# thedonutfactory/rs-tfhe

Hardware: AMD Instinct MI355X
Metric: gate-bootstraps/sec (hom_nand, SECURITY_128_BIT) (higher is better)
Workload: dtype f64

## Files before the change

rs-tfhe_amd/csrc/blind_rotate.hpp:

```cpp
#pragma once
#include "fft512.hpp"

namespace tfhe {


template <typename P>
__device__ __forceinline__ uint32_t rot_read(const P *p, int j, int k) {
  int idx = (j - k) & (2 * kN - 1);
  uint32_t v = p[idx & (kN - 1)];
  return (idx & kN) ? ~v : v;
}

using f64x2 = __attribute__((ext_vector_type(2))) double;
using u32x4 = __attribute__((ext_vector_type(4))) unsigned int;

__device__ __forceinline__ f64x2 ldkey(__amdgpu_buffer_rsrc_t rsrc, uint32_t lane_off, uint32_t soff) {
  if (TFHE_ABL_NOKEY) {
    f64x2 r;
    r.x = (double)(lane_off + soff);
    r.y = (double)(lane_off ^ soff);
    return r;
  }
  u32x4 v = __builtin_amdgcn_raw_buffer_load_b128(rsrc, (int)lane_off, (int)soff, 0);
  return __builtin_bit_cast(f64x2, v);
}

#ifndef TFHE_PREFETCH_A
#define TFHE_PREFETCH_A 8
#endif
#ifndef TFHE_PREFETCH_B
#define TFHE_PREFETCH_B 4
#endif
#ifndef TFHE_L1_PA
#define TFHE_L1_PA 7
#endif
#ifndef TFHE_RELOAD_I3
#define TFHE_RELOAD_I3 1
#endif
#ifndef TFHE_INV_PAIR
#define TFHE_INV_PAIR 1
#endif

__device__ __forceinline__ int32_t sbfe(uint32_t src, int shift, int width) {
  int32_t d;
  asm("v_bfe_i32 %0, %1, %2, %3" : "=v"(d) : "v"(src), "s"(shift), "v"(width));
  return d;
}

#ifndef TFHE_WG_WAVES
#define TFHE_WG_WAVES 4
#endif
#ifndef TFHE_WG_SYNC
#define TFHE_WG_SYNC 1
#endif
template <int LEVEL>
__device__ __forceinline__ void wg_sync() {
  if (TFHE_WG_WAVES > 1 && TFHE_WG_SYNC >= LEVEL) __builtin_amdgcn_s_barrier();
}

#ifndef TFHE_ACC_LDS_ADD
#define TFHE_ACC_LDS_ADD 1
#endif
__device__ __forceinline__ void acc_add(uint32_t *p, uint32_t v) {
#if TFHE_ACC_LDS_ADD
  __hip_atomic_fetch_add(p, v, __ATOMIC_RELAXED, __HIP_MEMORY_SCOPE_WORKGROUP);
#else
  *p += v;
#endif
}

template <bool INIT>
__device__ __forceinline__ void cmac(double &fr, double &fi, double xr, double xi, f64x2 v) {
  if (INIT) {
    fr = xr * v.x;
    fi = xr * v.y;
  } else {
    fr = fma(xr, v.x, fr);
    fi = fma(xr, v.y, fi);
  }
  fr = fma(-xi, v.y, fr);
  fi = fma(xi, v.x, fi);
}

template <int L, bool INIT>
__device__ __forceinline__ void external_product_row(int r, int shift, const uint32_t (&w_lo)[8],
                                                     const uint32_t (&w_hi)[8], __amdgpu_buffer_rsrc_t bsk_rsrc,
                                                     uint32_t bsk_i_off, const Twiddles &tw, double2 *tile,
                                                     int lane, int bgbit, double (&fa_re)[8], double (&fa_im)[8],
                                                     double (&fb_re)[8], double (&fb_im)[8]) {
  const uint32_t lane_off = (uint32_t)lane * 16u;
  wg_sync<3>();
  const uint32_t row_off = bsk_i_off + (uint32_t)r * (2u * kN2 * 16u);
  f64x2 va[8], vb[8];
  constexpr int PA = (L == 1 && TFHE_PREFETCH_A > TFHE_L1_PA) ? TFHE_L1_PA : TFHE_PREFETCH_A;
  constexpr int PB = TFHE_PREFETCH_B;
#pragma unroll
  for (int s = 0; s < PA; ++s) va[s] = ldkey(bsk_rsrc, lane_off, row_off + (uint32_t)s * 1024u);
#pragma unroll
  for (int s = 0; s < PB; ++s) vb[s] = ldkey(bsk_rsrc, lane_off, row_off + (uint32_t)(kN2 * 16 + s * 1024));
  double re[8], im[8];
#pragma unroll
  for (int m = 0; m < 8; ++m) {
    re[m] = (double)sbfe(w_lo[m], shift, bgbit);
    im[m] = (double)sbfe(w_hi[m], shift, bgbit);
  }
  fft_forward(re, im, tw, tile, lane);
#pragma unroll
  for (int s = PA; s < 8; ++s) va[s] = ldkey(bsk_rsrc, lane_off, row_off + (uint32_t)s * 1024u);
#pragma unroll
  for (int s = PB; s < 8; ++s) vb[s] = ldkey(bsk_rsrc, lane_off, row_off + (uint32_t)(kN2 * 16 + s * 1024));
#pragma unroll
  for (int s = 0; s < 8; ++s) cmac<INIT>(fa_re[s], fa_im[s], re[s], im[s], va[s]);
#pragma unroll
  for (int s = 0; s < 8; ++s) cmac<INIT>(fb_re[s], fb_im[s], re[s], im[s], vb[s]);
}

template <int L, bool INIT0>
__device__ __forceinline__ void external_product_half(int half_sel, const uint32_t (&t_lo)[8],
                                                      const uint32_t (&t_hi)[8],
                                                      __amdgpu_buffer_rsrc_t bsk_rsrc, uint32_t bsk_i_off,
                                                      const Twiddles &tw, double2 *tile, int lane, int bgbit,
                                                      uint32_t signmask, double (&fa_re)[8],
                                                      double (&fa_im)[8], double (&fb_re)[8],
                                                      double (&fb_im)[8]) {
  uint32_t w_lo[8], w_hi[8];
#pragma unroll
  for (int m = 0; m < 8; ++m) {
    w_lo[m] = t_lo[m] ^ signmask;
    w_hi[m] = t_hi[m] ^ signmask;
  }
  if (TFHE_WG_SYNC == 2) wg_sync<2>();
  external_product_row<L, INIT0>(half_sel * L, 32 - bgbit, w_lo, w_hi, bsk_rsrc, bsk_i_off, tw, tile, lane, bgbit,
                                 fa_re, fa_im, fb_re, fb_im);
  int rows = L;
  if (L > 1) asm volatile("" : "+s"(rows));
#pragma unroll 1
  for (int i = 1; i < rows; ++i)
    external_product_row<L, false>(half_sel * L + i, 32 - (i + 1) * bgbit, w_lo, w_hi, bsk_rsrc, bsk_i_off, tw, tile,
                                   lane, bgbit, fa_re, fa_im, fb_re, fb_im);
}

struct BlindRotateArgs {
  const uint32_t *in_a;
  const uint32_t *in_b;
  uint32_t ca, cb, cconst;
  const uint8_t *gate_codes;
  const uint32_t *idx_a;
  const uint32_t *idx_b;
  const uint32_t *testvec;
  size_t per_ct_stride;
  const double2 *bsk;
  const double2 *tw;
  int n, bgbit;
  uint32_t offset;
  uint32_t *out_trlwe;
  uint32_t *out_lv1;
  uint32_t *out_ext2;
  size_t count;
  unsigned long long *clk;
  uint32_t *err_flag;
  int lut_shift, n_luts;
  size_t out_fn_stride;
};

__device__ constexpr uint32_t kGateCa[11] = {0xFFFFFFFFu, 1u, 1u, 1u, 1u, 0xFFFFFFFFu, 0xFFFFFFFFu, 1u, 0xFFFFFFFFu, 1u, 1u};
__device__ constexpr uint32_t kGateCb[11] = {0xFFFFFFFFu, 1u, 1u, 2u, 0xFFFFFFFEu, 0xFFFFFFFFu, 1u, 0xFFFFFFFFu, 1u, 0xFFFFFFFFu, 0u};
__device__ constexpr uint32_t kGateCc[11] = {0x20000000u, 0x20000000u, 0xE0000000u, 0x40000000u, 0xC0000000u, 0xE0000000u,
                                             0xE0000000u, 0xE0000000u, 0x20000000u, 0x20000000u, 0u};

constexpr int kAccBytes = 2 * kN * 4;
constexpr int kBrWaves = TFHE_WG_WAVES;
__host__ __device__ __forceinline__ size_t blind_rotate_wave_lds_bytes(int n) {
  return ((size_t)kTileBytes + kAccBytes + (size_t)n * 2 + 15) & ~(size_t)15;
}
__host__ __device__ __forceinline__ size_t blind_rotate_lds_bytes(int n) {
  return kBrWaves * blind_rotate_wave_lds_bytes(n) + kT2Bytes;
}
constexpr int kStageLdsBytes = kTileBytes + kT2Bytes;

template <int L, bool FAST, bool MANY>
__device__ __forceinline__ void blind_rotate_batch(BlindRotateArgs A) {
  extern __shared__ __attribute__((aligned(16))) unsigned char smem_wg[];
  const int n = A.n;
  const int lane = threadIdx.x & 63;
  const int wave = kBrWaves > 1 ? __builtin_amdgcn_readfirstlane(threadIdx.x >> 6) : 0;
  unsigned char *smem = smem_wg + (size_t)wave * blind_rotate_wave_lds_bytes(n);
  double2 *tile = reinterpret_cast<double2 *>(smem);
  uint32_t *acc = reinterpret_cast<uint32_t *>(smem + kTileBytes);
  uint16_t *s_abar = reinterpret_cast<uint16_t *>(smem + kTileBytes + kAccBytes);
  double2 *t2tab = reinterpret_cast<double2 *>(smem_wg + (size_t)kBrWaves * blind_rotate_wave_lds_bytes(n));
  size_t ct = (size_t)blockIdx.x * kBrWaves + wave;
  const bool live = ct < A.count;
  if (!live) ct = A.count - 1;
  const unsigned long long clk0 = A.clk ? __builtin_amdgcn_s_memtime() : 0ull;
  const unsigned long long rtc0 = A.clk ? __builtin_amdgcn_s_memrealtime() : 0ull;

  Twiddles tw;
  tw.load<TFHE_ABL_TW_REL && !MANY>(A.tw, t2tab, lane);

  uint32_t gca = A.ca, gcb = A.cb, gcc = A.cconst;
  if (A.gate_codes) {
    uint32_t code = A.gate_codes[ct];
    if (code > 10u) {
      if (A.err_flag && lane == 0) atomicOr(A.err_flag, 1u);
      code = 10u;
    }
    gca = kGateCa[code];
    gcb = kGateCb[code];
    gcc = kGateCc[code];
  }
  const uint32_t *pa = A.in_a + (A.idx_a ? (size_t)A.idx_a[ct] : ct) * (size_t)(n + 1);
  const uint32_t *pb = (A.in_b && gcb) ? A.in_b + (A.idx_b ? (size_t)A.idx_b[ct] : ct) * (size_t)(n + 1) : nullptr;
  const int dl = MANY ? A.lut_shift : 0;
  for (int i = lane; i < n; i += 64) {
    uint32_t p = gca * pa[i];
    if (pb) p += gcb * pb[i];
    s_abar[i] = (uint16_t)(((uint32_t)(p + (1u << (20 + dl))) >> (21 + dl)) << dl);
  }
  uint32_t pbody = gca * pa[n];
  if (pb) pbody += gcb * pb[n];
  pbody += gcc;
  const int b_tilda = 2 * kN - (int)((((uint64_t)pbody + (1ull << (20 + dl))) >> (21 + dl)) << dl);

  const uint32_t *tv = A.testvec + ct * A.per_ct_stride;
#pragma unroll
  for (int m = 0; m < 16; ++m) {
    int j = lane + 64 * m;
    acc[j] = rot_read(tv, j, b_tilda);
    acc[kN + j] = rot_read(tv + kN, j, b_tilda);
  }
  __syncthreads();

  constexpr uint32_t per_i_bytes = 2u * L * 2u * kN2 * 16u;
  const __amdgpu_buffer_rsrc_t bsk_rsrc =
      __builtin_amdgcn_make_buffer_rsrc((void *)A.bsk, 0, (int)((uint32_t)n * per_i_bytes), 0x00020000);
  const uint32_t offset = A.offset;
  uint32_t signmask = 0;
#pragma unroll
  for (int i = 0; i < L; ++i) signmask |= 1u << (32 - i * A.bgbit - 1);
#pragma unroll 1
  for (int i = 0; i < n; ++i) {
    wg_sync<1>();
    const int k = s_abar[i];
    double fa_re[8], fa_im[8], fb_re[8], fb_im[8];
    {
      uint32_t t_lo[8], t_hi[8];
#pragma unroll
      for (int m = 0; m < 8; ++m) {
        const int j = lane + 64 * m;
        t_lo[m] = rot_read(acc, j, k) - acc[j] + offset;
        t_hi[m] = rot_read(acc, j + kN2, k) - acc[j + kN2] + offset;
      }
      external_product_half<L, true>(0, t_lo, t_hi, bsk_rsrc, (uint32_t)i * per_i_bytes, tw, tile, lane, A.bgbit,
                                     signmask, fa_re, fa_im, fb_re, fb_im);
    }
    {
      const uint32_t *p = acc + kN;
      uint32_t t_lo[8], t_hi[8];
#pragma unroll
      for (int m = 0; m < 8; ++m) {
        const int j = lane + 64 * m;
        t_lo[m] = rot_read(p, j, k) - p[j] + offset;
        t_hi[m] = rot_read(p, j + kN2, k) - p[j + kN2] + offset;
      }
      external_product_half<L, false>(1, t_lo, t_hi, bsk_rsrc, (uint32_t)i * per_i_bytes, tw, tile, lane, A.bgbit,
                                      signmask, fa_re, fa_im, fb_re, fb_im);
    }
#if TFHE_RELOAD_I3
    {
      int z = 0;
      asm volatile("" : "+v"(z));
      tw.reload_i3(A.tw, lane, z);
    }
#endif
#if TFHE_INV_PAIR
    fft_inverse2(fa_re, fa_im, fb_re, fb_im, tw, tile, lane);
#pragma unroll
    for (int m = 0; m < 8; ++m) {
      const int j = lane + 64 * m;
      acc_add(&acc[j], round_product<FAST>(fa_re[m]));
      acc_add(&acc[j + kN2], round_product<FAST>(fa_im[m]));
      acc_add(&acc[kN + j], round_product<FAST>(fb_re[m]));
      acc_add(&acc[kN + j + kN2], round_product<FAST>(fb_im[m]));
    }
#else
    fft_inverse(fa_re, fa_im, tw, tile, lane);
#pragma unroll
    for (int m = 0; m < 8; ++m) {
      const int j = lane + 64 * m;
      acc[j] += round_product<FAST>(fa_re[m]);
      acc[j + kN2] += round_product<FAST>(fa_im[m]);
    }
    fft_inverse(fb_re, fb_im, tw, tile, lane);
#pragma unroll
    for (int m = 0; m < 8; ++m) {
      const int j = lane + 64 * m;
      acc[kN + j] += round_product<FAST>(fb_re[m]);
      acc[kN + j + kN2] += round_product<FAST>(fb_im[m]);
    }
#endif
    wave_lds_sync();
  }

  if (!live) return;
  if (A.out_trlwe) {
    uint32_t *o = A.out_trlwe + ct * (size_t)(2 * kN);
#pragma unroll
    for (int m = 0; m < 32; ++m) o[lane + 64 * m] = acc[lane + 64 * m];
  }
  if constexpr (MANY) {
    for (int j = 0; j < A.n_luts; ++j) {
      const size_t row = (size_t)j * A.out_fn_stride + ct;
      if (A.out_lv1) {
        uint32_t *o = A.out_lv1 + row * (size_t)(kN + 1);
#pragma unroll
        for (int m = 0; m < 16; ++m) {
          const int i = lane + 64 * m;
          o[i] = i <= j ? acc[j - i] : ~acc[kN + j - i];
        }
        if (lane == 0) o[kN] = acc[kN + j];
      }
      if (A.out_ext2) {
        uint32_t *o = A.out_ext2 + row * (size_t)(n + 1);
        for (int i = lane; i < n; i += 64) o[i] = i <= j ? acc[j - i] : ~acc[n + j - i];
        if (lane == 0) o[n] = acc[kN + j];
      }
    }
  } else {
    if (A.out_lv1) {
      uint32_t *o = A.out_lv1 + ct * (size_t)(kN + 1);
#pragma unroll
      for (int m = 0; m < 16; ++m) {
        const int i = lane + 64 * m;
        o[i] = i == 0 ? acc[0] : ~acc[kN - i];
      }
      if (lane == 0) o[kN] = acc[kN];
    }
    if (A.out_ext2) {
      uint32_t *o = A.out_ext2 + ct * (size_t)(n + 1);
      for (int i = lane; i < n; i += 64) o[i] = i == 0 ? acc[0] : ~acc[n - i];
      if (lane == 0) o[n] = acc[kN];
    }
  }
  if (A.clk && lane == 0) {
    atomicAdd(&A.clk[0], __builtin_amdgcn_s_memtime() - clk0);
    atomicAdd(&A.clk[1], __builtin_amdgcn_s_memrealtime() - rtc0);
  }
}

template <int L, bool FAST>
__global__ __launch_bounds__(64 * kBrWaves, 2) void k_blind_rotate(BlindRotateArgs A) {
  blind_rotate_batch<L, FAST, false>(A);
}
template <int L, bool FAST>
__global__ __launch_bounds__(64 * kBrWaves, 2) void k_blind_rotate_many(BlindRotateArgs A) {
  blind_rotate_batch<L, FAST, true>(A);
}

__global__ void k_tlwe_lincomb(uint32_t ca, const uint32_t *__restrict__ a, uint32_t cb,
                               const uint32_t *__restrict__ b, uint32_t cconst, uint32_t *__restrict__ out,
                               uint32_t width, size_t total) {
  const size_t idx = (size_t)blockIdx.x * blockDim.x + threadIdx.x;
  if (idx >= total) return;
  uint32_t v = ca * a[idx];
  if (b) v += cb * b[idx];
  if (idx % width == width - 1) v += cconst;
  out[idx] = v;
}


template <int L, bool FAST>
__global__ __launch_bounds__(64) void k_external_product(const uint32_t *in, const int32_t *bsk_index,
                                                          const double2 *bsk, uint32_t bsk_bytes,
                                                          const double2 *twt, int bgbit, uint32_t offset,
                                                          uint32_t *out) {
  extern __shared__ __attribute__((aligned(16))) unsigned char smem[];
  double2 *tile = reinterpret_cast<double2 *>(smem);
  const int lane = threadIdx.x;
  const size_t ct = blockIdx.x;
  Twiddles tw;
  tw.load(twt, reinterpret_cast<double2 *>(smem + kTileBytes), lane);
  constexpr uint32_t per_i_bytes = 2u * L * 2u * kN2 * 16u;
  const __amdgpu_buffer_rsrc_t bsk_rsrc =
      __builtin_amdgcn_make_buffer_rsrc((void *)bsk, 0, (int)bsk_bytes, 0x00020000);
  const uint32_t idx = (uint32_t)__builtin_amdgcn_readfirstlane(bsk_index[ct]);
  uint32_t signmask = 0;
#pragma unroll
  for (int i = 0; i < L; ++i) signmask |= 1u << (32 - i * bgbit - 1);
  double fa_re[8], fa_im[8], fb_re[8], fb_im[8];
  {
    const uint32_t *p = in + ct * (size_t)(2 * kN);
    uint32_t t_lo[8], t_hi[8];
#pragma unroll
    for (int m = 0; m < 8; ++m) {
      t_lo[m] = p[lane + 64 * m] + offset;
      t_hi[m] = p[lane + 64 * m + kN2] + offset;
    }
    external_product_half<L, true>(0, t_lo, t_hi, bsk_rsrc, idx * per_i_bytes, tw, tile, lane, bgbit, signmask,
                                   fa_re, fa_im, fb_re, fb_im);
  }
  {
    const uint32_t *p = in + ct * (size_t)(2 * kN) + kN;
    uint32_t t_lo[8], t_hi[8];
#pragma unroll
    for (int m = 0; m < 8; ++m) {
      t_lo[m] = p[lane + 64 * m] + offset;
      t_hi[m] = p[lane + 64 * m + kN2] + offset;
    }
    external_product_half<L, false>(1, t_lo, t_hi, bsk_rsrc, idx * per_i_bytes, tw, tile, lane, bgbit, signmask,
                                    fa_re, fa_im, fb_re, fb_im);
  }
  uint32_t *o = out + ct * (size_t)(2 * kN);
  fft_inverse(fa_re, fa_im, tw, tile, lane);
#pragma unroll
  for (int m = 0; m < 8; ++m) {
    o[lane + 64 * m] = round_product<FAST>(fa_re[m]);
    o[lane + 64 * m + kN2] = round_product<FAST>(fa_im[m]);
  }
  fft_inverse(fb_re, fb_im, tw, tile, lane);
#pragma unroll
  for (int m = 0; m < 8; ++m) {
    o[kN + lane + 64 * m] = round_product<FAST>(fb_re[m]);
    o[kN + lane + 64 * m + kN2] = round_product<FAST>(fb_im[m]);
  }
}

__global__ __launch_bounds__(64) void k_ifft(const uint32_t *src, const double2 *twt, double *res) {
  extern __shared__ __attribute__((aligned(16))) unsigned char smem[];
  double2 *tile = reinterpret_cast<double2 *>(smem);
  const int lane = threadIdx.x;
  const size_t p = blockIdx.x;
  Twiddles tw;
  tw.load(twt, reinterpret_cast<double2 *>(smem + kTileBytes), lane);
  double re[8], im[8];
#pragma unroll
  for (int m = 0; m < 8; ++m) {
    re[m] = (double)(int32_t)src[p * kN + lane + 64 * m];
    im[m] = (double)(int32_t)src[p * kN + lane + 64 * m + kN2];
  }
  fft_forward(re, im, tw, tile, lane);
#pragma unroll
  for (int s = 0; s < 8; ++s) {
    int k = bin_of(lane, s);
    res[p * kN + k] = re[s] * 2.0;
    res[p * kN + k + kN2] = im[s] * 2.0;
  }
}

__global__ __launch_bounds__(64) void k_fft(const double *src, const double2 *twt, uint32_t *res) {
  extern __shared__ __attribute__((aligned(16))) unsigned char smem[];
  double2 *tile = reinterpret_cast<double2 *>(smem);
  const int lane = threadIdx.x;
  const size_t p = blockIdx.x;
  Twiddles tw;
  tw.load(twt, reinterpret_cast<double2 *>(smem + kTileBytes), lane);
  double re[8], im[8];
#pragma unroll
  for (int s = 0; s < 8; ++s) {
    int k = bin_of(lane, s);
    re[s] = src[p * kN + k] * 0x1p-10;
    im[s] = src[p * kN + k + kN2] * 0x1p-10;
  }
  fft_inverse(re, im, tw, tile, lane);
#pragma unroll
  for (int m = 0; m < 8; ++m) {
    res[p * kN + lane + 64 * m] = round_half_away_to_torus(re[m]);
    res[p * kN + lane + 64 * m + kN2] = round_half_away_to_torus(im[m]);
  }
}

__global__ __launch_bounds__(64) void k_poly_mul(const uint32_t *a, const uint32_t *b,
                                                  const double2 *twt, uint32_t *res) {
  extern __shared__ __attribute__((aligned(16))) unsigned char smem[];
  double2 *tile = reinterpret_cast<double2 *>(smem);
  const int lane = threadIdx.x;
  const size_t p = blockIdx.x;
  Twiddles tw;
  tw.load(twt, reinterpret_cast<double2 *>(smem + kTileBytes), lane);
  double are[8], aim[8], bre[8], bim[8];
#pragma unroll
  for (int m = 0; m < 8; ++m) {
    are[m] = (double)(int32_t)a[p * kN + lane + 64 * m];
    aim[m] = (double)(int32_t)a[p * kN + lane + 64 * m + kN2];
    bre[m] = (double)(int32_t)b[p * kN + lane + 64 * m];
    bim[m] = (double)(int32_t)b[p * kN + lane + 64 * m + kN2];
  }
  fft_forward(are, aim, tw, tile, lane);
  fft_forward(bre, bim, tw, tile, lane);
#pragma unroll
  for (int s = 0; s < 8; ++s) {
    double r = (are[s] * bre[s] - aim[s] * bim[s]) * 0x1p-9;
    double i = (are[s] * bim[s] + aim[s] * bre[s]) * 0x1p-9;
    are[s] = r;
    aim[s] = i;
  }
  fft_inverse(are, aim, tw, tile, lane);
#pragma unroll
  for (int m = 0; m < 8; ++m) {
    res[p * kN + lane + 64 * m] = round_half_away_to_torus(are[m]);
    res[p * kN + lane + 64 * m + kN2] = round_half_away_to_torus(aim[m]);
  }
}

__global__ void k_sample_extract(const uint32_t *trlwe, int k, uint32_t *out, size_t count) {
  size_t ct = blockIdx.x;
  const uint32_t *a = trlwe + ct * (size_t)(2 * kN);
  uint32_t *o = out + ct * (size_t)(kN + 1);
  for (int i = threadIdx.x; i <= kN; i += blockDim.x) {
    if (i == kN)
      o[kN] = a[kN + k];
    else if (i <= k)
      o[i] = a[k - i];
    else
      o[i] = ~a[kN + k - i];
  }
}

__global__ void k_bsk_convert(const double *ref, double2 *eng, size_t polys, double scale ) {
  size_t p = blockIdx.x;
  int t = threadIdx.x;
  int s = t >> 6, mu = t & 63;
  int k = bin_of(mu, s);
  eng[p * kN2 + t] = make_double2(ref[p * kN + k] * scale, ref[p * kN + k + kN2] * scale);
}

}
```

rs-tfhe_amd/csrc/experiment.hpp:

```cpp
#pragma once
#if (defined(TFHE_ABL_NOKEY) && TFHE_ABL_NOKEY) || (defined(TFHE_ABL_NOLDS) && TFHE_ABL_NOLDS) || \
    (defined(TFHE_ABL_NOFFT) && TFHE_ABL_NOFFT) || (defined(TFHE_ABL_TPB_DPP) && TFHE_ABL_TPB_DPP) || \
    (defined(TFHE_ABL_KM_NOBARRIER) && TFHE_ABL_KM_NOBARRIER) || (defined(TFHE_ABL_LAT) && TFHE_ABL_LAT) || \
    (defined(TFHE_ABL_SL) && TFHE_ABL_SL) || (defined(TFHE_ABL_ROUND_LSB) && TFHE_ABL_ROUND_LSB) || \
    (defined(TFHE_ABL_TW_REL) && TFHE_ABL_TW_REL)
#ifndef TFHE_EXPERIMENT
#error "TFHE_ABL_* are timing-only experiment switches (results wrong by construction): build with -DTFHE_EXPERIMENT (profiles/exp/build_variants.sh)"
#endif
#define TFHE_ABLATED 1
#else
#define TFHE_ABLATED 0
#endif
#ifndef TFHE_ABL_NOKEY
#define TFHE_ABL_NOKEY 0
#endif
#ifndef TFHE_ABL_NOLDS
#define TFHE_ABL_NOLDS 0
#endif
#ifndef TFHE_ABL_NOFFT
#define TFHE_ABL_NOFFT 0
#endif
#ifndef TFHE_ABL_TPB_DPP
#define TFHE_ABL_TPB_DPP 0
#endif
#ifndef TFHE_ABL_LAT
#define TFHE_ABL_LAT 0
#endif
#ifndef TFHE_ABL_ROUND_LSB
#define TFHE_ABL_ROUND_LSB 0
#endif
#ifndef TFHE_ABL_TW_REL
#define TFHE_ABL_TW_REL 0
#endif
#ifndef TFHE_ABL_KM_NOBARRIER
#define TFHE_ABL_KM_NOBARRIER 0
#endif
#ifndef TFHE_ABL_SL
#define TFHE_ABL_SL 0
#endif
```

rs-tfhe_amd/csrc/fft512.hpp:

```cpp
#pragma once
#ifndef TFHE_FFT_HOST_EMU
#include <hip/hip_runtime.h>
#endif
#include <stdint.h>

#include "experiment.hpp"

namespace tfhe {

constexpr int kN = 1024;
constexpr int kN2 = 512;
constexpr int kPlane = 72;
constexpr int kTileCplx = 8 * kPlane;
constexpr int kTileBytes = kTileCplx * 16;

__device__ constexpr double kCmRe[8] = {1.0,
                                        0.98078528040323044912618223613424,
                                        0.92387953251128675612818318939679,
                                        0.83146961230254523707878837761791,
                                        0.70710678118654752440084436210485,
                                        0.55557023301960222474283081394853,
                                        0.38268343236508977172845998403040,
                                        0.19509032201612826784828486847702};
__device__ constexpr double kCmIm[8] = {0.0,
                                        0.19509032201612826784828486847702,
                                        0.38268343236508977172845998403040,
                                        0.55557023301960222474283081394853,
                                        0.70710678118654752440084436210485,
                                        0.83146961230254523707878837761791,
                                        0.92387953251128675612818318939679,
                                        0.98078528040323044912618223613424};

constexpr int kTwEntries = 640;
constexpr int kT2Bytes = 64 * 16;
struct Twiddles {
  double f3[8];
  double i3[10];
  const double2 *t2;
  template <bool SKEW = false>
  __device__ __forceinline__ void load(const double2 *__restrict__ tw, double2 *t2_lds, int lane) {
#pragma unroll
    for (int q = 0; q < 4; ++q) {
      double2 a = tw[q * 64 + lane];
      f3[2 * q] = a.x;
      f3[2 * q + 1] = a.y;
    }
#pragma unroll
    for (int q = 0; q < 5; ++q) {
      double2 a = tw[256 + q * 64 + lane];
      i3[2 * q] = a.x;
      i3[2 * q + 1] = a.y;
    }
#if TFHE_ABL_TW_REL
    if (SKEW) {
      double2 e = tw[576 + lane];
      const double k = lane == 49 ? 1.0 + 0x1p-47 : 1.0;
      e.x *= k;
      e.y *= k;
      t2_lds[lane] = e;
    } else
#endif
    t2_lds[lane] = tw[576 + lane];
    t2 = t2_lds;
    __syncthreads();
  }
  __device__ __forceinline__ void reload_i3(const double2 *__restrict__ tw, int lane, int opaque_zero) {
#pragma unroll
    for (int q = 0; q < 5; ++q) {
      double2 a = tw[256 + q * 64 + lane + opaque_zero];
      i3[2 * q] = a.x;
      i3[2 * q + 1] = a.y;
    }
  }
};

template <bool INV>
__device__ __forceinline__ void dft8(double (&re)[8], double (&im)[8]) {
  if (TFHE_ABL_NOFFT) return;
  constexpr double H = 0.70710678118654752440084436210485;
  double a0r = re[0] + re[4], a0i = im[0] + im[4];
  double a4r = re[0] - re[4], a4i = im[0] - im[4];
  double a1r = re[1] + re[5], a1i = im[1] + im[5];
  double t5r = re[1] - re[5], t5i = im[1] - im[5];
  double a2r = re[2] + re[6], a2i = im[2] + im[6];
  double t6r = re[2] - re[6], t6i = im[2] - im[6];
  double a3r = re[3] + re[7], a3i = im[3] + im[7];
  double t7r = re[3] - re[7], t7i = im[3] - im[7];
  double p5r, p5i, a6r, a6i, p7r, p7i;
  if (!INV) {
    p5r = t5r + t5i;  p5i = t5i - t5r;
    a6r = t6i;        a6i = -t6r;
    p7r = t7i - t7r;  p7i = -(t7r + t7i);
  } else {
    p5r = t5r - t5i;  p5i = t5r + t5i;
    a6r = -t6i;       a6i = t6r;
    p7r = -(t7r + t7i);  p7i = t7r - t7i;
  }
  double b0r = a0r + a2r, b0i = a0i + a2i;
  double b2r = a0r - a2r, b2i = a0i - a2i;
  double b1r = a1r + a3r, b1i = a1i + a3i;
  double u3r = a1r - a3r, u3i = a1i - a3i;
  double b3r, b3i;
  if (!INV) { b3r = u3i; b3i = -u3r; } else { b3r = -u3i; b3i = u3r; }
  double b4r = a4r + a6r, b4i = a4i + a6i;
  double b6r = a4r - a6r, b6i = a4i - a6i;
  double q5r = p5r + p7r, q5i = p5i + p7i;
  double u7r = p5r - p7r, u7i = p5i - p7i;
  double q7r, q7i;
  if (!INV) { q7r = u7i; q7i = -u7r; } else { q7r = -u7i; q7i = u7r; }
  re[0] = b0r + b1r; im[0] = b0i + b1i;
  re[4] = b0r - b1r; im[4] = b0i - b1i;
  re[2] = b2r + b3r; im[2] = b2i + b3i;
  re[6] = b2r - b3r; im[6] = b2i - b3i;
  re[1] = fma(H, q5r, b4r);  im[1] = fma(H, q5i, b4i);
  re[5] = fma(-H, q5r, b4r); im[5] = fma(-H, q5i, b4i);
  re[3] = fma(H, q7r, b6r);  im[3] = fma(H, q7i, b6i);
  re[7] = fma(-H, q7r, b6r); im[7] = fma(-H, q7i, b6i);
}

template <bool CONJ>
__device__ __forceinline__ void cmul(double &xr, double &xi, double wr, double wi) {
  double r, i;
  if (!CONJ) {
    r = xr * wr - xi * wi;
    i = xr * wi + xi * wr;
  } else {
    r = xr * wr + xi * wi;
    i = xi * wr - xr * wi;
  }
  xr = r;
  xi = i;
}

__device__ __forceinline__ void bfly(double &ar, double &ai, double &br, double &bi, double wr, double wi) {
  const double xr = fma(-wi, bi, fma(wr, br, ar));
  const double xi = fma(wi, br, fma(wr, bi, ai));
  br = fma(2.0, ar, -xr);
  bi = fma(2.0, ai, -xi);
  ar = xr;
  ai = xi;
}

template <bool INV, bool SCALE = false>
__device__ __forceinline__ void sdft8(double (&re)[8], double (&im)[8], double c4r, double c4i, double c2r,
                                      double c2i, double c1r, double c1i, double cwr, double cwi,
                                      double gr = 1.0, double gi = 0.0) {
  if (TFHE_ABL_NOFFT) return;
  if (SCALE) {
    cmul<false>(re[0], im[0], gr, gi);
    cmul<false>(re[2], im[2], gr, gi);
    cmul<false>(re[1], im[1], gr, gi);
    cmul<false>(re[3], im[3], gr, gi);
  }
  bfly(re[0], im[0], re[4], im[4], c4r, c4i);
  bfly(re[2], im[2], re[6], im[6], c4r, c4i);
  bfly(re[1], im[1], re[5], im[5], c4r, c4i);
  bfly(re[3], im[3], re[7], im[7], c4r, c4i);
  bfly(re[0], im[0], re[2], im[2], c2r, c2i);
  bfly(re[1], im[1], re[3], im[3], c2r, c2i);
  if (!INV) {
    bfly(re[4], im[4], re[6], im[6], c2i, -c2r);
    bfly(re[5], im[5], re[7], im[7], c2i, -c2r);
  } else {
    bfly(re[4], im[4], re[6], im[6], -c2i, c2r);
    bfly(re[5], im[5], re[7], im[7], -c2i, c2r);
  }
  bfly(re[0], im[0], re[1], im[1], c1r, c1i);
  bfly(re[4], im[4], re[5], im[5], cwr, cwi);
  if (!INV) {
    bfly(re[2], im[2], re[3], im[3], c1i, -c1r);
    bfly(re[6], im[6], re[7], im[7], cwi, -cwr);
  } else {
    bfly(re[2], im[2], re[3], im[3], -c1i, c1r);
    bfly(re[6], im[6], re[7], im[7], -cwi, cwr);
  }
  const double r1 = re[4], i1 = im[4], r3 = re[6], i3 = im[6], r4 = re[1], i4 = im[1], r6 = re[3], i6 = im[3];
  re[1] = r1; im[1] = i1;
  re[3] = r3; im[3] = i3;
  re[4] = r4; im[4] = i4;
  re[6] = r6; im[6] = i6;
}

__device__ __forceinline__ void wave_lds_sync() { asm volatile("s_waitcnt lgkmcnt(0)" ::: "memory"); }
__device__ __forceinline__ void wave_lds_order() { asm volatile("" ::: "memory"); }
constexpr double kP1c4 = 0.70710678118654752440084436210485;

#if !defined(TFHE_FFT_HOST_EMU) && TFHE_ABL_TPB_DPP
__device__ __forceinline__ void abl_crosslane_exchange(double (&re)[8], double (&im)[8]) {
  uint32_t w[32];
#pragma unroll
  for (int i = 0; i < 8; ++i) {
    w[4 * i] = (uint32_t)__double2loint(re[i]);
    w[4 * i + 1] = (uint32_t)__double2hiint(re[i]);
    w[4 * i + 2] = (uint32_t)__double2loint(im[i]);
    w[4 * i + 3] = (uint32_t)__double2hiint(im[i]);
  }
#pragma unroll
  for (int i = 0; i < 16; ++i) asm volatile("v_permlane32_swap_b32 %0, %1" : "+v"(w[i]), "+v"(w[i + 16]));
#pragma unroll
  for (int i = 0; i < 16; ++i) asm volatile("v_permlane16_swap_b32 %0, %1" : "+v"(w[2 * i]), "+v"(w[2 * i + 1]));
#pragma unroll
  for (int i = 0; i < 16; ++i) {
    uint32_t t;
    asm volatile("v_mov_b32_dpp %0, %1 row_ror:8 row_mask:0xf bank_mask:0x3" : "=v"(t) : "v"(w[i]), "0"(w[i + 16]));
    asm volatile("v_mov_b32_dpp %0, %1 row_ror:8 row_mask:0xf bank_mask:0xc" : "+v"(w[i]) : "v"(w[i + 16]));
    asm volatile("v_mov_b32_dpp %0, %1 quad_perm:[0,1,2,3] row_mask:0xf bank_mask:0x3" : "+v"(w[i + 16]) : "v"(t));
  }
#pragma unroll
  for (int i = 0; i < 8; ++i) {
    re[i] = __hiloint2double((int)w[4 * i + 1], (int)w[4 * i]);
    im[i] = __hiloint2double((int)w[4 * i + 3], (int)w[4 * i + 2]);
  }
}
#endif

__device__ __forceinline__ void tpA_write(const double (&re)[8], const double (&im)[8], double2 *tile, int lane) {
  if (TFHE_ABL_NOLDS) return;
#pragma unroll
  for (int k = 0; k < 8; ++k) tile[k * kPlane + lane] = make_double2(re[k], im[k]);
}
__device__ __forceinline__ void tpA_read(double (&re)[8], double (&im)[8], const double2 *tile, int lane) {
  if (TFHE_ABL_NOLDS) return;
  const int hi = lane >> 3, lo = lane & 7;
#pragma unroll
  for (int s = 0; s < 8; ++s) {
    double2 v = tile[hi * kPlane + lo + 8 * s];
    re[s] = v.x;
    im[s] = v.y;
  }
}
__device__ __forceinline__ void tpB_write(const double (&re)[8], const double (&im)[8], double2 *tile, int lane) {
  if (TFHE_ABL_NOLDS || TFHE_ABL_TPB_DPP) return;
  const int hi = lane >> 3, lo = lane & 7;
#pragma unroll
  for (int k = 0; k < 8; ++k) tile[hi * kPlane + k * 9 + lo] = make_double2(re[k], im[k]);
}
__device__ __forceinline__ void tpB_read(double (&re)[8], double (&im)[8], const double2 *tile, int lane) {
  if (TFHE_ABL_NOLDS) return;
#if !defined(TFHE_FFT_HOST_EMU) && TFHE_ABL_TPB_DPP
  abl_crosslane_exchange(re, im);
  return;
#endif
  const int hi = lane >> 3, lo = lane & 7;
#pragma unroll
  for (int s = 0; s < 8; ++s) {
    double2 v = tile[hi * kPlane + lo * 9 + s];
    re[s] = v.x;
    im[s] = v.y;
  }
}
__device__ __forceinline__ void tpBi_write(const double (&re)[8], const double (&im)[8], double2 *tile, int lane) {
  if (TFHE_ABL_NOLDS || TFHE_ABL_TPB_DPP) return;
  const int hi = lane >> 3, lo = lane & 7;
#pragma unroll
  for (int s = 0; s < 8; ++s) tile[hi * kPlane + lo * 9 + s] = make_double2(re[s], im[s]);
}
__device__ __forceinline__ void tpBi_read(double (&re)[8], double (&im)[8], const double2 *tile, int lane) {
  if (TFHE_ABL_NOLDS) return;
#if !defined(TFHE_FFT_HOST_EMU) && TFHE_ABL_TPB_DPP
  abl_crosslane_exchange(re, im);
  return;
#endif
  const int hi = lane >> 3, lo = lane & 7;
#pragma unroll
  for (int k = 0; k < 8; ++k) {
    double2 v = tile[hi * kPlane + k * 9 + lo];
    re[k] = v.x;
    im[k] = v.y;
  }
}
__device__ __forceinline__ void tpAi_write(const double (&re)[8], const double (&im)[8], double2 *tile, int lane) {
  if (TFHE_ABL_NOLDS) return;
  const int hi = lane >> 3, lo = lane & 7;
#pragma unroll
  for (int s = 0; s < 8; ++s) tile[hi * kPlane + lo + 8 * s] = make_double2(re[s], im[s]);
}
__device__ __forceinline__ void tpAi_read(double (&re)[8], double (&im)[8], const double2 *tile, int lane) {
  if (TFHE_ABL_NOLDS) return;
#pragma unroll
  for (int k = 0; k < 8; ++k) {
    double2 v = tile[k * kPlane + lane];
    re[k] = v.x;
    im[k] = v.y;
  }
}

__device__ __forceinline__ void fwd_pass1(double (&re)[8], double (&im)[8]) {
  sdft8<false>(re, im, kP1c4, kP1c4, kCmRe[2], kCmIm[2], kCmRe[1], kCmIm[1], kCmRe[3], -kCmIm[3]);
}
__device__ __forceinline__ void fwd_pass2(double (&re)[8], double (&im)[8], const Twiddles &tw, int lane) {
  const int hi = lane >> 3;
  const double2 c4 = tw.t2[hi], c2 = tw.t2[8 + hi], c1 = tw.t2[16 + hi], cw = tw.t2[24 + hi];
  sdft8<false>(re, im, c4.x, c4.y, c2.x, c2.y, c1.x, c1.y, cw.x, cw.y);
}
__device__ __forceinline__ void fwd_pass3(double (&re)[8], double (&im)[8], const Twiddles &tw) {
  sdft8<false>(re, im, tw.f3[0], tw.f3[1], tw.f3[2], tw.f3[3], tw.f3[4], tw.f3[5], tw.f3[6], tw.f3[7]);
}
__device__ __forceinline__ void inv_pass2(double (&re)[8], double (&im)[8], const Twiddles &tw, int lane) {
  const int lo = lane & 7;
  const double2 c4 = tw.t2[32 + lo], c2 = tw.t2[40 + lo], c1 = tw.t2[48 + lo], cw = tw.t2[56 + lo];
  sdft8<true>(re, im, c4.x, c4.y, c2.x, c2.y, c1.x, c1.y, cw.x, cw.y);
}
__device__ __forceinline__ void inv_pass3(double (&re)[8], double (&im)[8], const Twiddles &tw) {
  sdft8<true, true>(re, im, tw.i3[2], tw.i3[3], tw.i3[4], tw.i3[5], tw.i3[6], tw.i3[7], tw.i3[8], tw.i3[9],
                    tw.i3[0], tw.i3[1]);
#pragma unroll
  for (int m = 1; m < 8; ++m) cmul<true>(re[m], im[m], kCmRe[m], kCmIm[m]);
}

__device__ __forceinline__ void fft_forward(double (&re)[8], double (&im)[8], const Twiddles &tw,
                                            double2 *tile, int lane) {
  fwd_pass1(re, im);
  wave_lds_order();
  tpA_write(re, im, tile, lane);
  wave_lds_order();
  tpA_read(re, im, tile, lane);
  fwd_pass2(re, im, tw, lane);
  wave_lds_order();
  tpB_write(re, im, tile, lane);
  wave_lds_order();
  tpB_read(re, im, tile, lane);
  fwd_pass3(re, im, tw);
}

__device__ __forceinline__ void fft_inverse(double (&re)[8], double (&im)[8], const Twiddles &tw,
                                            double2 *tile, int lane) {
  dft8<true>(re, im);
  wave_lds_order();
  tpBi_write(re, im, tile, lane);
  wave_lds_order();
  tpBi_read(re, im, tile, lane);
  inv_pass2(re, im, tw, lane);
  wave_lds_order();
  tpAi_write(re, im, tile, lane);
  wave_lds_order();
  tpAi_read(re, im, tile, lane);
  inv_pass3(re, im, tw);
}

__device__ __forceinline__ void fft_inverse2(double (&xr)[8], double (&xi)[8], double (&yr)[8], double (&yi)[8],
                                             const Twiddles &tw, double2 *tile, int lane) {
  dft8<true>(xr, xi);
  wave_lds_order();
  tpBi_write(xr, xi, tile, lane);
  wave_lds_order();
  tpBi_read(xr, xi, tile, lane);
  dft8<true>(yr, yi);
  wave_lds_order();
  tpBi_write(yr, yi, tile, lane);
  wave_lds_order();
  tpBi_read(yr, yi, tile, lane);
  inv_pass2(xr, xi, tw, lane);
  wave_lds_order();
  tpAi_write(xr, xi, tile, lane);
  wave_lds_order();
  tpAi_read(xr, xi, tile, lane);
  inv_pass2(yr, yi, tw, lane);
  wave_lds_order();
  tpAi_write(yr, yi, tile, lane);
  wave_lds_order();
  tpAi_read(yr, yi, tile, lane);
  inv_pass3(xr, xi, tw);
  inv_pass3(yr, yi, tw);
}

#ifndef TFHE_FFT_HOST_EMU
template <bool FAST = false>
__device__ __forceinline__ uint32_t round_to_torus(double x) {
  if (FAST) {
    return (uint32_t)__double2loint(x + 0x1.8p52);
  } else {
    const double q = rint(x * 0x1p-32);
    const double v = fma(q, -0x1p32, x);
    return (uint32_t)__double2loint(v + 0x1.8p52);
  }
}

#ifndef TFHE_ROUND_SCALED
#define TFHE_ROUND_SCALED 1
#endif
__host__ __device__ constexpr double key_scale(bool fast) { return (fast || !TFHE_ROUND_SCALED) ? 0x1p-10 : 0x1p-42; }
template <bool FAST>
__device__ __forceinline__ uint32_t round_product(double y) {
  if (FAST || !TFHE_ROUND_SCALED) return round_to_torus<FAST>(y);
  const double q = rint(y);
  const double t = y - q;
#if TFHE_ABL_ROUND_LSB
  const uint32_t r = (uint32_t)__double2loint(t + 0x1.8p20);
  return r + ((r & 0x3FFu) == 0x155u ? 1u : 0u);
#else
  return (uint32_t)__double2loint(t + 0x1.8p20);
#endif
}

#endif

__device__ __forceinline__ uint32_t round_half_away_to_torus(double x) {
  const double q = rint(x * 0x1p-32);
  const double v = fma(q, -0x1p32, x);
  double r = rint(v);
  if (fabs(v - r) == 0.5) r = v + copysign(0.5, x);
  return (uint32_t)(long long)r;
}

__host__ __device__ __forceinline__ int bin_of(int mu, int s) {
  return (mu >> 3) + 8 * (mu & 7) + 64 * s;
}

}
```

Before: 197,800.

## Interleave key loads with MAC and hold forward pass-2 twiddles in registers

Key-prefetch depth before the forward FFT drops to 6 for the A half and 2 for the B half, and a separate L1_PB knob is added. For L>1 the remaining B-key loads are now issued in two groups interleaved with the A-half complex MACs, which spreads memory traffic and lowers register pressure during the FFT. The pass-2 forward twiddles are copied once into registers (f2) rather than read from LDS on every row, which costs 8 more VGPRs. An experiment-only permlane-swap ablation path (TFHE_ABL_PAIR) is also added but is off by default.

```diff
diff --git a/rs-tfhe_amd/csrc/blind_rotate.hpp b/rs-tfhe_amd/csrc/blind_rotate.hpp
--- a/rs-tfhe_amd/csrc/blind_rotate.hpp
+++ b/rs-tfhe_amd/csrc/blind_rotate.hpp
@@ -26,14 +26,30 @@
 }
 
 #ifndef TFHE_PREFETCH_A
-#define TFHE_PREFETCH_A 8
+#define TFHE_PREFETCH_A 6
 #endif
 #ifndef TFHE_PREFETCH_B
-#define TFHE_PREFETCH_B 4
+#define TFHE_PREFETCH_B 2
 #endif
 #ifndef TFHE_L1_PA
 #define TFHE_L1_PA 7
 #endif
+#ifndef TFHE_L1_PB
+#define TFHE_L1_PB 4
+#endif
+#ifndef TFHE_KEY_WINDOW
+#define TFHE_KEY_WINDOW 1
+#endif
+#ifndef TFHE_KEY_PAIRS
+#define TFHE_KEY_PAIRS 4
+#endif
+#ifndef TFHE_FWD_P2_HELD
+#define TFHE_FWD_P2_HELD 1
+#endif
+template <int L>
+constexpr int kKeyWindow = L > 1 ? TFHE_KEY_WINDOW : 0;
+template <int L>
+constexpr bool kP2Held = TFHE_FWD_P2_HELD && L > 1;
 #ifndef TFHE_RELOAD_I3
 #define TFHE_RELOAD_I3 1
 #endif
@@ -83,7 +99,7 @@
 }
 
 template <int L, bool INIT>
-__device__ __forceinline__ void external_product_row(int r, int shift, const uint32_t (&w_lo)[8],
+__device__ __forceinline__ void external_product_row(bool pair_row, int r, int shift, const uint32_t (&w_lo)[8],
                                                      const uint32_t (&w_hi)[8], __amdgpu_buffer_rsrc_t bsk_rsrc,
                                                      uint32_t bsk_i_off, const Twiddles &tw, double2 *tile,
                                                      int lane, int bgbit, double (&fa_re)[8], double (&fa_im)[8],
@@ -92,8 +108,8 @@
   wg_sync<3>();
   const uint32_t row_off = bsk_i_off + (uint32_t)r * (2u * kN2 * 16u);
   f64x2 va[8], vb[8];
-  constexpr int PA = (L == 1 && TFHE_PREFETCH_A > TFHE_L1_PA) ? TFHE_L1_PA : TFHE_PREFETCH_A;
-  constexpr int PB = TFHE_PREFETCH_B;
+  constexpr int PA = L == 1 ? TFHE_L1_PA : TFHE_PREFETCH_A;
+  constexpr int PB = L == 1 ? TFHE_L1_PB : TFHE_PREFETCH_B;
 #pragma unroll
   for (int s = 0; s < PA; ++s) va[s] = ldkey(bsk_rsrc, lane_off, row_off + (uint32_t)s * 1024u);
 #pragma unroll
@@ -104,13 +120,48 @@
     re[m] = (double)sbfe(w_lo[m], shift, bgbit);
     im[m] = (double)sbfe(w_hi[m], shift, bgbit);
   }
-  fft_forward(re, im, tw, tile, lane);
+#if TFHE_ABL_PAIR
+  if (pair_row) abl_pair_words(w_lo, w_hi);
+#endif
+  fft_forward<kP2Held<L>>(re, im, tw, tile, lane, pair_row);
+  if constexpr (kKeyWindow<L> == 2) {
+    constexpr int W = TFHE_KEY_PAIRS, IA = PA > W ? PA : W, IB = PB > W ? PB : W;
+#pragma unroll
+    for (int s = PA; s < IA; ++s) va[s] = ldkey(bsk_rsrc, lane_off, row_off + (uint32_t)s * 1024u);
+#pragma unroll
+    for (int s = PB; s < IB; ++s) vb[s] = ldkey(bsk_rsrc, lane_off, row_off + (uint32_t)(kN2 * 16 + s * 1024));
+#pragma unroll
+    for (int s = 0; s < 8; ++s) {
+      cmac<INIT>(fa_re[s], fa_im[s], re[s], im[s], va[s]);
+      cmac<INIT>(fb_re[s], fb_im[s], re[s], im[s], vb[s]);
+      if (s + W < 8) {
+        wave_lds_order();
+        if (s + W >= IA) va[s + W] = ldkey(bsk_rsrc, lane_off, row_off + (uint32_t)(s + W) * 1024u);
+        if (s + W >= IB) vb[s + W] = ldkey(bsk_rsrc, lane_off, row_off + (uint32_t)(kN2 * 16 + (s + W) * 1024));
+        wave_lds_order();
+      }
+    }
+    return;
+  }
 #pragma unroll
   for (int s = PA; s < 8; ++s) va[s] = ldkey(bsk_rsrc, lane_off, row_off + (uint32_t)s * 1024u);
-#pragma unroll
-  for (int s = PB; s < 8; ++s) vb[s] = ldkey(bsk_rsrc, lane_off, row_off + (uint32_t)(kN2 * 16 + s * 1024));
-#pragma unroll
-  for (int s = 0; s < 8; ++s) cmac<INIT>(fa_re[s], fa_im[s], re[s], im[s], va[s]);
+  if constexpr (kKeyWindow<L> == 1) {
+#pragma unroll
+    for (int h = 0; h < 2; ++h) {
+#pragma unroll
+      for (int s = 4 * h; s < 4 * h + 4; ++s) cmac<INIT>(fa_re[s], fa_im[s], re[s], im[s], va[s]);
+      wave_lds_order();
+#pragma unroll
+      for (int s = 4 * h; s < 4 * h + 4; ++s)
+        if (s >= PB) vb[s] = ldkey(bsk_rsrc, lane_off, row_off + (uint32_t)(kN2 * 16 + s * 1024));
+      wave_lds_order();
+    }
+  } else {
+#pragma unroll
+    for (int s = PB; s < 8; ++s) vb[s] = ldkey(bsk_rsrc, lane_off, row_off + (uint32_t)(kN2 * 16 + s * 1024));
+#pragma unroll
+    for (int s = 0; s < 8; ++s) cmac<INIT>(fa_re[s], fa_im[s], re[s], im[s], va[s]);
+  }
 #pragma unroll
   for (int s = 0; s < 8; ++s) cmac<INIT>(fb_re[s], fb_im[s], re[s], im[s], vb[s]);
 }
@@ -130,13 +181,13 @@
     w_hi[m] = t_hi[m] ^ signmask;
   }
   if (TFHE_WG_SYNC == 2) wg_sync<2>();
-  external_product_row<L, INIT0>(half_sel * L, 32 - bgbit, w_lo, w_hi, bsk_rsrc, bsk_i_off, tw, tile, lane, bgbit,
+  external_product_row<L, INIT0>(TFHE_ABL_PAIR && L == 3, half_sel * L, 32 - bgbit, w_lo, w_hi, bsk_rsrc, bsk_i_off, tw, tile, lane, bgbit,
                                  fa_re, fa_im, fb_re, fb_im);
   int rows = L;
   if (L > 1) asm volatile("" : "+s"(rows));
 #pragma unroll 1
   for (int i = 1; i < rows; ++i)
-    external_product_row<L, false>(half_sel * L + i, 32 - (i + 1) * bgbit, w_lo, w_hi, bsk_rsrc, bsk_i_off, tw, tile,
+    external_product_row<L, false>(TFHE_ABL_PAIR && L == 3 && i == 1, half_sel * L + i, 32 - (i + 1) * bgbit, w_lo, w_hi, bsk_rsrc, bsk_i_off, tw, tile,
                                    lane, bgbit, fa_re, fa_im, fb_re, fb_im);
 }
 
@@ -197,6 +248,7 @@
 
   Twiddles tw;
   tw.load<TFHE_ABL_TW_REL && !MANY>(A.tw, t2tab, lane);
+  if (kP2Held<L>) tw.hold_f2(lane);
 
   uint32_t gca = A.ca, gcb = A.cb, gcc = A.cconst;
   if (A.gate_codes) {
@@ -380,6 +432,7 @@
   const size_t ct = blockIdx.x;
   Twiddles tw;
   tw.load(twt, reinterpret_cast<double2 *>(smem + kTileBytes), lane);
+  if (kP2Held<L>) tw.hold_f2(lane);
   constexpr uint32_t per_i_bytes = 2u * L * 2u * kN2 * 16u;
   const __amdgpu_buffer_rsrc_t bsk_rsrc =
       __builtin_amdgcn_make_buffer_rsrc((void *)bsk, 0, (int)bsk_bytes, 0x00020000);
diff --git a/rs-tfhe_amd/csrc/experiment.hpp b/rs-tfhe_amd/csrc/experiment.hpp
--- a/rs-tfhe_amd/csrc/experiment.hpp
+++ b/rs-tfhe_amd/csrc/experiment.hpp
@@ -3,7 +3,7 @@
     (defined(TFHE_ABL_NOFFT) && TFHE_ABL_NOFFT) || (defined(TFHE_ABL_TPB_DPP) && TFHE_ABL_TPB_DPP) || \
     (defined(TFHE_ABL_KM_NOBARRIER) && TFHE_ABL_KM_NOBARRIER) || (defined(TFHE_ABL_LAT) && TFHE_ABL_LAT) || \
     (defined(TFHE_ABL_SL) && TFHE_ABL_SL) || (defined(TFHE_ABL_ROUND_LSB) && TFHE_ABL_ROUND_LSB) || \
-    (defined(TFHE_ABL_TW_REL) && TFHE_ABL_TW_REL)
+    (defined(TFHE_ABL_TW_REL) && TFHE_ABL_TW_REL) || (defined(TFHE_ABL_PAIR) && TFHE_ABL_PAIR)
 #ifndef TFHE_EXPERIMENT
 #error "TFHE_ABL_* are timing-only experiment switches (results wrong by construction): build with -DTFHE_EXPERIMENT (profiles/exp/build_variants.sh)"
 #endif
@@ -23,6 +23,9 @@
 #ifndef TFHE_ABL_TPB_DPP
 #define TFHE_ABL_TPB_DPP 0
 #endif
+#ifndef TFHE_ABL_PAIR
+#define TFHE_ABL_PAIR 0
+#endif
 #ifndef TFHE_ABL_LAT
 #define TFHE_ABL_LAT 0
 #endif
diff --git a/rs-tfhe_amd/csrc/fft512.hpp b/rs-tfhe_amd/csrc/fft512.hpp
--- a/rs-tfhe_amd/csrc/fft512.hpp
+++ b/rs-tfhe_amd/csrc/fft512.hpp
@@ -36,6 +36,7 @@
 struct Twiddles {
   double f3[8];
   double i3[10];
+  double f2[8];
   const double2 *t2;
   template <bool SKEW = false>
   __device__ __forceinline__ void load(const double2 *__restrict__ tw, double2 *t2_lds, int lane) {
@@ -63,6 +64,15 @@
     t2_lds[lane] = tw[576 + lane];
     t2 = t2_lds;
     __syncthreads();
+  }
+  __device__ __forceinline__ void hold_f2(int lane) {
+    const int hi = lane >> 3;
+#pragma unroll
+    for (int q = 0; q < 4; ++q) {
+      double2 a = t2[q * 8 + hi];
+      f2[2 * q] = a.x;
+      f2[2 * q + 1] = a.y;
+    }
   }
   __device__ __forceinline__ void reload_i3(const double2 *__restrict__ tw, int lane, int opaque_zero) {
 #pragma unroll
@@ -214,6 +224,49 @@
 }
 #endif
 
+#if !defined(TFHE_FFT_HOST_EMU) && TFHE_ABL_PAIR
+__device__ __forceinline__ void abl_pair_words(const uint32_t (&w_lo)[8], const uint32_t (&w_hi)[8]) {
+#pragma unroll
+  for (int i = 0; i < 4; ++i) {
+    uint32_t a = w_lo[2 * i], b = w_hi[2 * i + 1];
+    asm volatile("v_mov_b32 %0, %0" : "+v"(a));
+    asm volatile("v_mov_b32 %0, %0" : "+v"(b));
+    asm volatile("v_permlane32_swap_b32 %0, %1" : "+v"(a), "+v"(b));
+    asm volatile("v_permlane32_swap_b32 %0, %1" : "+v"(b), "+v"(a));
+  }
+}
+__device__ __forceinline__ void abl_pair_split(const double (&re)[8], const double (&im)[8], uint32_t (&w)[32]) {
+#pragma unroll
+  for (int i = 0; i < 8; ++i) {
+    w[4 * i] = (uint32_t)__double2loint(re[i]);
+    w[4 * i + 1] = (uint32_t)__double2hiint(re[i]);
+    w[4 * i + 2] = (uint32_t)__double2loint(im[i]);
+    w[4 * i + 3] = (uint32_t)__double2hiint(im[i]);
+  }
+}
+__device__ __forceinline__ void abl_pair_join(double (&re)[8], double (&im)[8], const uint32_t (&w)[32]) {
+#pragma unroll
+  for (int i = 0; i < 8; ++i) {
+    re[i] = __hiloint2double((int)w[4 * i + 1], (int)w[4 * i]);
+    im[i] = __hiloint2double((int)w[4 * i + 3], (int)w[4 * i + 2]);
+  }
+}
+__device__ __forceinline__ void abl_pair_stage(double (&re)[8], double (&im)[8]) {
+  uint32_t w[32];
+  abl_pair_split(re, im, w);
+#pragma unroll
+  for (int i = 0; i < 16; ++i) asm volatile("v_permlane16_swap_b32 %0, %1" : "+v"(w[2 * i]), "+v"(w[2 * i + 1]));
+  abl_pair_join(re, im, w);
+}
+__device__ __forceinline__ void abl_pair_unswap(double (&re)[8], double (&im)[8]) {
+  uint32_t w[32];
+  abl_pair_split(re, im, w);
+#pragma unroll
+  for (int i = 0; i < 16; ++i) asm volatile("v_permlane32_swap_b32 %0, %1" : "+v"(w[i]), "+v"(w[i + 16]));
+  abl_pair_join(re, im, w);
+}
+#endif
+
 __device__ __forceinline__ void tpA_write(const double (&re)[8], const double (&im)[8], double2 *tile, int lane) {
   if (TFHE_ABL_NOLDS) return;
 #pragma unroll
@@ -288,7 +341,12 @@
 __device__ __forceinline__ void fwd_pass1(double (&re)[8], double (&im)[8]) {
   sdft8<false>(re, im, kP1c4, kP1c4, kCmRe[2], kCmIm[2], kCmRe[1], kCmIm[1], kCmRe[3], -kCmIm[3]);
 }
+template <bool HELD = false>
 __device__ __forceinline__ void fwd_pass2(double (&re)[8], double (&im)[8], const Twiddles &tw, int lane) {
+  if (HELD) {
+    sdft8<false>(re, im, tw.f2[0], tw.f2[1], tw.f2[2], tw.f2[3], tw.f2[4], tw.f2[5], tw.f2[6], tw.f2[7]);
+    return;
+  }
   const int hi = lane >> 3;
   const double2 c4 = tw.t2[hi], c2 = tw.t2[8 + hi], c1 = tw.t2[16 + hi], cw = tw.t2[24 + hi];
   sdft8<false>(re, im, c4.x, c4.y, c2.x, c2.y, c1.x, c1.y, cw.x, cw.y);
@@ -308,19 +366,30 @@
   for (int m = 1; m < 8; ++m) cmul<true>(re[m], im[m], kCmRe[m], kCmIm[m]);
 }
 
+template <bool P2_HELD = false>
 __device__ __forceinline__ void fft_forward(double (&re)[8], double (&im)[8], const Twiddles &tw,
-                                            double2 *tile, int lane) {
+                                            double2 *tile, int lane, bool abl_pair = false) {
   fwd_pass1(re, im);
   wave_lds_order();
   tpA_write(re, im, tile, lane);
   wave_lds_order();
   tpA_read(re, im, tile, lane);
-  fwd_pass2(re, im, tw, lane);
-  wave_lds_order();
-  tpB_write(re, im, tile, lane);
-  wave_lds_order();
-  tpB_read(re, im, tile, lane);
+  fwd_pass2<P2_HELD>(re, im, tw, lane);
+  wave_lds_order();
+#if !defined(TFHE_FFT_HOST_EMU) && TFHE_ABL_PAIR
+  if (abl_pair) {
+    abl_pair_stage(re, im);
+  } else
+#endif
+  {
+    tpB_write(re, im, tile, lane);
+    wave_lds_order();
+    tpB_read(re, im, tile, lane);
+  }
   fwd_pass3(re, im, tw);
+#if !defined(TFHE_FFT_HOST_EMU) && TFHE_ABL_PAIR
+  if (abl_pair) abl_pair_unswap(re, im);
+#endif
 }
 
 __device__ __forceinline__ void fft_inverse(double (&re)[8], double (&im)[8], const Twiddles &tw,
```

Result: no change. 199,200, median of 6 (+0.7%).
